# abodthedude25/Ray_Tracing_Octrees

Hardware: AMD Instinct MI355X
Metric: Mrays/s (primary rays), 1920x1080 (higher is better)
Workload: dtype f32

## Files before the change

### ray_tracing_octrees_amd/csrc/rto_device.hip.h

```cpp
#pragma once

#include <hip/hip_runtime.h>
#include <stdint.h>

#include "../../include/rto_hip.h"

namespace rto {

constexpr int kMaxTraversalSteps = 512;
constexpr int kWave = 64;
#ifndef RTO_BLOCK
#define RTO_BLOCK 256
#endif
constexpr int kBlock = RTO_BLOCK;
#ifndef RTO_PACKED3_WAVES
#define RTO_PACKED3_WAVES 6
#endif
#ifndef RTO_PERSIST_CHUNK
#define RTO_PERSIST_CHUNK 8
#endif
constexpr int kMaxDepth = 20;
constexpr int kStackCap = 7 * kMaxDepth + 1;

struct StartState {
// ... 819 lines not shown
    int lvl = 0;
    unsigned lvlPending = 0;
    unsigned tailRun = 0;

#if defined(RTO_STAMP)
    unsigned long long stampSum[5] = { 0, 0, 0, 0, 0 };
#define RTO_T(i) do { __builtin_amdgcn_sched_barrier(0); unsigned long long t_; asm volatile("s_memtime %0\n\ts_waitcnt lgkmcnt(0)" : "=s"(t_) :: "memory"); __builtin_amdgcn_sched_barrier(0); stampSum[i] += t_ - stampLast; stampLast = t_; } while (0)
    unsigned long long stampLast;
    asm volatile("s_memtime %0\n\ts_waitcnt lgkmcnt(0)" : "=s"(stampLast) :: "memory");
#else
#define RTO_T(i) do { } while (0)
#endif
    int trips = 0;
    while (alive) {
        trips++;
        if (MODE == kModeTimeline) tlIters++;
        RTO_T(4);
        const uint2 d = desc[cur];
        const int L = 31 - __builtin_clz(lvlPending | 1u);
        const uint2 e = stk[L * kWave];
        const int half = 1 << (P.depth - 1 - lvl);
        unsigned passMask;
        if (anyRisky) passMask = child_pass_mask<true>(P, r, cx, cy, cz, half);
        else passMask = child_pass_mask_fast(P, r, cx, cy, cz, half);
        RTO_T(0);
        const unsigned vm0 = __builtin_amdgcn_ubfe(d.x, 16, 8);
        const unsigned im0 = __builtin_amdgcn_ubfe(d.x, 8, 8);
        const unsigned sm = d.x & vm0;
        unsigned cand = ((im0 & vm0) | sm) & passMask;
#if defined(RTO_STAMP)
        asm volatile("" :: "v"(cand));
#endif
        RTO_T(1);
        const unsigned solidHit = sm & passMask;
        cand &= 0xffffffffu << (31 - __builtin_clz(solidHit | 1u));
        const bool noWork = cand == 0;
        const int stepsB = steps + __builtin_popcount(vm0) + (int)tailRun;
        const bool dead = noWork && (lvlPending == 0 || stepsB >= kMaxTraversalSteps);
        steps = noWork ? stepsB : steps;
        const unsigned W = noWork ? e.x : ((d.x & 0x00ffff00u) | cand | (tailRun << 24));
        const unsigned base = noWork ? e.y : d.y;
#if defined(RTO_STAMP)
        asm volatile("" :: "v"(W), "v"(base));
#endif
        RTO_T(2);
        const int lvl2 = noWork ? L : lvl;
        const int bpos = P.depth - 1 - lvl2;
        const unsigned childIdx = ((cx >> bpos) & 1) | (((cy >> bpos) & 1) << 1) | (((cz >> bpos) & 1) << 2);
        const unsigned belowPrev = noWork ? ((1u << childIdx) - 1u) : 0xffu;
        const int keep = (int)(0xffffffffu << (bpos + 1));
        cx &= keep; cy &= keep; cz &= keep;
        const unsigned pending = W & 0xffu;
        const unsigned im = __builtin_amdgcn_ubfe(W, 8, 8);
        const unsigned vm = __builtin_amdgcn_ubfe(W, 16, 8);
        const unsigned tailAbove = W >> 24;
        const int j = 31 - __builtin_clz(pending | 1u);
        const unsigned bitj = 1u << j;
        const int stepsC = steps + __builtin_popcount(vm & belowPrev & ~((bitj << 1) - 1u));
        const bool capped = stepsC >= kMaxTraversalSteps;
        const bool go = !dead && !capped;
        const bool solid = (im & bitj) == 0;
        steps = dead ? steps : (capped ? kMaxTraversalSteps : stepsC + 1);
        hit = go && solid;
        const bool descend = go && !solid;
        if (descend) stk[lvl2 * kWave] = make_uint2(W ^ bitj, base);
        const unsigned pendingNew = pending ^ bitj;
        const unsigned lb = 1u << lvl2;
        tailRun = pendingNew ? 0u : tailAbove + (unsigned)__builtin_popcount(vm & (bitj - 1u));
        lvlPending = pendingNew ? (lvlPending | lb) : (lvlPending & ~lb);
        cur = base + (unsigned)__builtin_popcount(im & (bitj - 1u));
        const int hl = 1 << bpos;
        cx |= (j & 1) ? hl : 0; cy |= (j & 2) ? hl : 0; cz |= (j & 4) ? hl : 0;
        lvl = lvl2 + 1;
        alive = descend;
#if defined(RTO_STAMP)
        asm volatile("" :: "v"(cur), "v"(cx), "v"(lvlPending), "v"(tailRun));
#endif
        RTO_T(3);
    }
    if (!hit && steps > kMaxTraversalSteps) steps = kMaxTraversalSteps;
    trips = __builtin_amdgcn_readlane(wave_scan_max_nonneg(trips), kWave - 1);
    if (P.tileCost && lane == 0 && ty < P.tilesY) P.tileCost[tile] = trips;

    const bool mine = valid && !(P.skipOutside && outsideRoot);
    if (MODE == kModeShade) {
        if (mine) __builtin_nontemporal_store(hit ? shade_term(P, r, cx, cy, cz, P.rootSize >> lvl) : kShadeMiss, reinterpret_cast<float*>(out) + (size_t)ly * P.W + px);
        fill_outside<MODE>(P, out, lane, slot);
    } else if (MODE == kModeColor || MODE == kModeTimeline) {
        if (mine) {
            float4 color = make_float4(0.f, 0.f, 0.f, 1.f);
            if (hit) color = shade_hit(P, r, cx, cy, cz, P.rootSize >> lvl);
            store_pixel(out + (size_t)ly * P.W + px, color);
        }
        fill_outside<MODE>(P, out, lane, slot);
        if (MODE == kModeTimeline) {
            int it = tlIters;
            for (int off = 32; off > 0; off >>= 1) it = max(it, __shfl_down(it, off));
            int act = __builtin_popcountll(__builtin_amdgcn_ballot_w64(tlIters > 0));
            if (lane == 0 && ty < P.tilesY) {
                const unsigned long long tl1 = wall_clock64();
                unsigned hwid = __builtin_amdgcn_s_getreg((4 << 0) | (0 << 6) | (31 << 11));
                unsigned xcc = __builtin_amdgcn_s_getreg((20 << 0) | (0 << 6) | (3 << 11));
                int* rec = stepsOut + (size_t)tile * 8;
                rec[0] = (int)(tl0 & 0xffffffffu); rec[1] = (int)(tl0 >> 32);
                rec[2] = (int)(tl1 & 0xffffffffu); rec[3] = (int)(tl1 >> 32);
                rec[4] = it; rec[5] = (int)hwid; rec[6] = (int)xcc; rec[7] = act;
#if defined(RTO_STAMP)
                rec[0] = (int)stampSum[0]; rec[1] = (int)stampSum[1]; rec[5] = (int)stampSum[2]; rec[6] = (int)stampSum[3]; rec[7] = (int)stampSum[4];
#endif
            }
        }
    } else {
        if (inImage) stepsOut[(size_t)py * P.W + px] = hit ? steps : -steps;
        wave_accumulate(counters, steps, hit, inImage);
    }
}

template <int MODE>
__global__ __launch_bounds__(kBlock, RTO_PACKED3_WAVES) void k_trace_packed3(RenderParams P, const uint2* __restrict__ desc,
                                                           float4* __restrict__ out, int* __restrict__ stepsOut,
                                                           Counters* __restrict__ counters) {
    extern __shared__ uint2 lds_stack[];
    const int lane = threadIdx.x & 63;
    const int wave = threadIdx.x >> 6;
    uint2* stk = lds_stack + (size_t)wave * P.depth * kWave + lane;
    const int slot = __builtin_amdgcn_readfirstlane(blockIdx.x * (kBlock / kWave) + wave);
    if (slot >= P.launchWaves) return;
    trace_tile_packed3<MODE>(P, desc, out, stepsOut, counters, stk, lane, slot);
}


template <int TT> __device__ __forceinline__ unsigned bop3(unsigned a, unsigned b, unsigned c) { return __builtin_amdgcn_bitop3_b32(a, b, c, TT); }
constexpr int kSelC = 0xD8;
constexpr int kAndOr = 0xEA;
constexpr int kOrAnd = 0xF8;
constexpr int kAndAndNot = 0x40;
constexpr int kReplace = 0x74;

constexpr unsigned kCoordBias = 0x4B000000u;
template <bool BIASED>
__device__ __forceinline__ void child_axis_terms(float g, float o, float inv, unsigned sgn, int c, float fh, float vs, float sv,
                                                 float& n0, float& n1, float& f0, float& f1) {
    const float fc = BIASED ? __uint_as_float((unsigned)c) - 8388608.0f : (float)c;
    const f32x2 fcc = (f32x2){ fc, fc } + (f32x2){ 0.0f, fh };
    const f32x2 lo = (f32x2){ g, g } + fcc * vs;
    const f32x2 hi = lo + sv;
    const f32x2 t1 = (lo - o) * inv;
    const f32x2 t2 = (hi - o) * inv;
    const unsigned a1x = __float_as_uint(t1.x), a2x = __float_as_uint(t2.x), a1y = __float_as_uint(t1.y), a2y = __float_as_uint(t2.y);
    n0 = __uint_as_float(bop3<kSelC>(a1x, a2x, sgn)); f0 = __uint_as_float(bop3<kSelC>(a2x, a1x, sgn));
    n1 = __uint_as_float(bop3<kSelC>(a1y, a2y, sgn)); f1 = __uint_as_float(bop3<kSelC>(a2y, a1y, sgn));
}

template <bool BIASED>
__device__ __forceinline__ void child_axis_terms_exact(float g, float o, float inv, unsigned sgn, int c, float fh, float vs, float sv,
                                                       float& n0, float& n1, float& f0, float& f1) {
    (void)fh;
    const float fc = BIASED ? __uint_as_float((unsigned)c) - 8388608.0f : (float)c;
    const float p0 = __builtin_fmaf(fc, vs, g);
    const float p1 = p0 + sv;
    const float p2 = p1 + sv;
    const f32x2 t01 = ((f32x2){ p0, p1 } - o) * inv;
    const float t2 = (p2 - o) * inv;
    const unsigned a0 = __float_as_uint(t01.x), a1 = __float_as_uint(t01.y), a2 = __float_as_uint(t2);
    n0 = __uint_as_float(bop3<kSelC>(a0, a1, sgn)); f0 = __uint_as_float(bop3<kSelC>(a1, a0, sgn));
    n1 = __uint_as_float(bop3<kSelC>(a1, a2, sgn)); f1 = __uint_as_float(bop3<kSelC>(a2, a1, sgn));
}

template <bool FOLD = true, bool BIASED = false, bool EXACT = false>
__device__ __forceinline__ unsigned child_fail_mask_fast(float gx, float gy, float gz, float vs, float ox, float oy, float oz,
                                                         float ix, float iy, float iz, unsigned sx, unsigned sy, unsigned sz,
                                                         int cx, int cy, int cz, float fh,
                                                         float clampLo = __uint_as_float(1u), float clampHi = __uint_as_float(0x7149f2c9u)) {
    const float sv = fh * vs;
    const float kEps = clampLo;
    const float kBelow1e30 = clampHi;
    float nx0, nx1, fx0, fx1, ny0, ny1, fy0, fy1, nz0, nz1, fz0, fz1;
    if (EXACT) {
        child_axis_terms_exact<BIASED>(gx, ox, ix, sx, cx, fh, vs, sv, nx0, nx1, fx0, fx1);
        child_axis_terms_exact<BIASED>(gy, oy, iy, sy, cy, fh, vs, sv, ny0, ny1, fy0, fy1);
        child_axis_terms_exact<BIASED>(gz, oz, iz, sz, cz, fh, vs, sv, nz0, nz1, fz0, fz1);
    } else {
        child_axis_terms<BIASED>(gx, ox, ix, sx, cx, fh, vs, sv, nx0, nx1, fx0, fx1);
        child_axis_terms<BIASED>(gy, oy, iy, sy, cy, fh, vs, sv, ny0, ny1, fy0, fy1);
        child_axis_terms<BIASED>(gz, oz, iz, sz, cz, fh, vs, sv, nz0, nz1, fz0, fz1);
    }
    if (FOLD) {
        asm("v_max_f32 %0, %1, %2" : "=v"(nx0) : "v"(nx0), "v"(kEps));
        asm("v_max_f32 %0, %1, %2" : "=v"(nx1) : "v"(nx1), "v"(kEps));
        asm("v_min_f32 %0, %1, %2" : "=v"(fx0) : "v"(fx0), "v"(kBelow1e30));
        asm("v_min_f32 %0, %1, %2" : "=v"(fx1) : "v"(fx1), "v"(kBelow1e30));
    }
#define RTO_D(kx, ky, kz) __float_as_uint(min3f(fx##kx, fy##ky, fz##kz) - max3f(nx##kx, ny##ky, nz##kz))
    unsigned fa = 0, fb = 0;
    fa = __builtin_amdgcn_alignbit(fa, RTO_D(1, 1, 1), 31); fb = __builtin_amdgcn_alignbit(fb, RTO_D(1, 1, 0), 31);
    fa = __builtin_amdgcn_alignbit(fa, RTO_D(0, 1, 1), 31); fb = __builtin_amdgcn_alignbit(fb, RTO_D(0, 1, 0), 31);
    fa = __builtin_amdgcn_alignbit(fa, RTO_D(1, 0, 1), 31); fb = __builtin_amdgcn_alignbit(fb, RTO_D(1, 0, 0), 31);
    fa = __builtin_amdgcn_alignbit(fa, RTO_D(0, 0, 1), 31); fb = __builtin_amdgcn_alignbit(fb, RTO_D(0, 0, 0), 31);
#undef RTO_D
    return (fa << 4) | fb;
}

struct ExactPat { unsigned kaX, kaY, kaZ, xXY, xXZ, xYZ; };
__device__ __forceinline__ ExactPat exact_patterns(unsigned sgnX, unsigned sgnY, unsigned sgnZ) {
    ExactPat p;
    p.kaX = 0xAAu ^ (sgnX & 0xFFu); p.kaY = 0xCCu ^ (sgnY & 0xFFu); p.kaZ = 0xF0u ^ (sgnZ & 0xFFu);
    p.xXY = p.kaX ^ p.kaY; p.xXZ = p.kaX ^ p.kaZ; p.xYZ = p.kaY ^ p.kaZ;
    return p;
}
constexpr int kOr3 = 0xFE;
template <bool BIASED>
__device__ __forceinline__ void axis_emx_exact(float g, float o, float inv, unsigned sgn, int c, float vs, float sv, float& e, float& m, float& x) {
    const float fc = BIASED ? __uint_as_float((unsigned)c) - 8388608.0f : (float)c;
    const float p0 = __builtin_fmaf(fc, vs, g);
    const float p1 = p0 + sv;
    const float p2 = p1 + sv;
    const f32x2 t02 = ((f32x2){ p0, p2 } - o) * inv;
    m = (p1 - o) * inv;
    const unsigned a0 = __float_as_uint(t02.x), a2 = __float_as_uint(t02.y);
    e = __uint_as_float(bop3<kSelC>(a0, a2, sgn)); x = __uint_as_float(bop3<kSelC>(a2, a0, sgn));
}
__device__ __forceinline__ unsigned fails_le(float u, float v) { return (unsigned)((int)__float_as_uint(v - u) >> 31); }

template <bool FOLD, bool BIASED>
__device__ __forceinline__ unsigned child_fail_mask_exactgrid(float gx, float gy, float gz, float vs, float ox, float oy, float oz,
                                                              float ix, float iy, float iz, unsigned sx, unsigned sy, unsigned sz, const ExactPat& K,
                                                              int cx, int cy, int cz, float fh,
                                                              float clampLo = __uint_as_float(1u), float clampHi = __uint_as_float(0x7149f2c9u)) {
    const float sv = fh * vs;
    float ex, mx, xx, ey, my, xy, ez, mz, xz;
    axis_emx_exact<BIASED>(gx, ox, ix, sx, cx, vs, sv, ex, mx, xx);
    axis_emx_exact<BIASED>(gy, oy, iy, sy, cy, vs, sv, ey, my, xy);
    axis_emx_exact<BIASED>(gz, oz, iz, sz, cz, vs, sv, ez, mz, xz);
    float Tn = max3f(ex, ey, ez), Tf = min3f(xx, xy, xz);
    if (FOLD) {
        asm("v_max_f32 %0, %1, %2" : "=v"(Tn) : "v"(Tn), "v"(clampLo));
        asm("v_min_f32 %0, %1, %2" : "=v"(Tf) : "v"(Tf), "v"(clampHi));
    }
    const unsigned selX = bop3<kSelC>(fails_le(Tn, mx), fails_le(mx, Tf), K.kaX);
    const unsigned selY = bop3<kSelC>(fails_le(Tn, my), fails_le(my, Tf), K.kaY);
    const unsigned selZ = bop3<kSelC>(fails_le(Tn, mz), fails_le(mz, Tf), K.kaZ);
    unsigned fail = bop3<kOr3>(selX, selY, selZ);
    const unsigned pXY = bop3<kSelC>(fails_le(my, mx), fails_le(mx, my), K.kaX);
    const unsigned pXZ = bop3<kSelC>(fails_le(mz, mx), fails_le(mx, mz), K.kaX);
    const unsigned pYZ = bop3<kSelC>(fails_le(mz, my), fails_le(my, mz), K.kaY);
    fail = bop3<kOrAnd>(fail, pXY, K.xXY);
    fail = bop3<kOrAnd>(fail, pXZ, K.xXZ);
    fail = bop3<kOrAnd>(fail, pYZ, K.xYZ);
    return fail;
}

struct ExactPat3 { unsigned pack; };
__device__ __forceinline__ ExactPat3 exact_patterns3(unsigned sgnX, unsigned sgnY, unsigned sgnZ) {
    ExactPat3 p;
    p.pack = (0xAAu ^ (sgnX & 0xFFu)) | ((0xCCu ^ (sgnY & 0xFFu)) << 8) | ((0xF0u ^ (sgnZ & 0xFFu)) << 16);
    return p;
}
constexpr int kAndXor = 0x60;
template <bool FOLD, bool BIASED>
__device__ __forceinline__ unsigned child_fail_mask_exactgrid3(float gx, float gy, float gz, float vs, float ox, float oy, float oz,
                                                               float ix, float iy, float iz, const ExactPat3& K,
                                                               int cx, int cy, int cz, float fh,
                                                               float clampLo = __uint_as_float(1u), float clampHi = __uint_as_float(0x7149f2c9u)) {
    const float sv = fh * vs;
    const unsigned sx = (unsigned)((int)__float_as_uint(ix) >> 31), sy = (unsigned)((int)__float_as_uint(iy) >> 31), sz = (unsigned)((int)__float_as_uint(iz) >> 31);
    float ex, mx, xx, ey, my, xy, ez, mz, xz;
    axis_emx_exact<BIASED>(gx, ox, ix, sx, cx, vs, sv, ex, mx, xx);
    axis_emx_exact<BIASED>(gy, oy, iy, sy, cy, vs, sv, ey, my, xy);
    axis_emx_exact<BIASED>(gz, oz, iz, sz, cz, vs, sv, ez, mz, xz);
    float Tn = max3f(ex, ey, ez), Tf = min3f(xx, xy, xz);
    if (FOLD) {
        asm("v_max_f32 %0, %1, %2" : "=v"(Tn) : "v"(Tn), "v"(clampLo));
        asm("v_min_f32 %0, %1, %2" : "=v"(Tf) : "v"(Tf), "v"(clampHi));
    }
    const unsigned kaX = K.pack, kaY = K.pack >> 8, kaZ = K.pack >> 16;
    const unsigned selX = bop3<kSelC>(fails_le(Tn, mx), fails_le(mx, Tf), kaX);
    const unsigned selY = bop3<kSelC>(fails_le(Tn, my), fails_le(my, Tf), kaY);
    const unsigned selZ = bop3<kSelC>(fails_le(Tn, mz), fails_le(mz, Tf), kaZ);
    const unsigned pXY = bop3<kAndXor>(bop3<kSelC>(fails_le(my, mx), fails_le(mx, my), kaX), kaX, kaY);
    const unsigned pXZ = bop3<kAndXor>(bop3<kSelC>(fails_le(mz, mx), fails_le(mx, mz), kaX), kaX, kaZ);
    const unsigned pYZ = bop3<kAndXor>(bop3<kSelC>(fails_le(mz, my), fails_le(my, mz), kaY), kaY, kaZ);
    return bop3<kOr3>(selX, selY, selZ) | bop3<kOr3>(pXY, pXZ, pYZ);
}

__device__ __forceinline__ unsigned child_fail_mask_exact(float gx, float gy, float gz, float vs, float ox, float oy, float oz,
                                                       float ix, float iy, float iz, int cx, int cy, int cz, int half) {
    const float sv = (float)half * vs;
    unsigned fail = 0;
#pragma unroll 1
    for (int k = 0; k < 8; k++) {
        const float mnx = gx + (float)(cx + ((k & 1) ? half : 0)) * vs;
        const float mny = gy + (float)(cy + ((k & 2) ? half : 0)) * vs;
        const float mnz = gz + (float)(cz + ((k & 4) ? half : 0)) * vs;
        const float t1x = (mnx - ox) * ix, t1y = (mny - oy) * iy, t1z = (mnz - oz) * iz;
        const float t2x = ((mnx + sv) - ox) * ix, t2y = ((mny + sv) - oy) * iy, t2z = ((mnz + sv) - oz) * iz;
        const float tn = gmax(gmax(gmin(t1x, t2x), gmin(t1y, t2y)), gmin(t1z, t2z));
        const float tf = gmin(gmin(gmax(t1x, t2x), gmax(t1y, t2y)), gmax(t1z, t2z));
        const bool ok = (tn <= tf) && (tf > 0.0f) && !(tn >= 1e30f);
        fail |= ok ? 0u : (1u << k);
    }
    return fail;
}

template <int MODE, int EXACT = -1>
__device__ __forceinline__ void trace_tile_lean(const RenderParams& P, const uint2* __restrict__ desc, float4* __restrict__ out,
                                                int* __restrict__ stepsOut, Counters* __restrict__ counters, uint2* stk,
                                                const int lane, const int slot) {
    unsigned long long tl0 = 0;
    if (MODE == kModeTimeline) tl0 = wall_clock64();

    int tile, tx, ty;
    resolve_slot(P, slot, tx, ty, tile);
    const int px = tx * 8 + (lane & 7);
    const int ly = ty * 8 + (lane >> 3);
    const bool valid = (ty < P.tilesY) && (px < P.W) && (ly < P.localRows);
    const int py = global_row(P, ly);
    const bool inImage = valid && (py < P.H);

    const Geo G = geo_of(P);
    bool hit = false;
    int steps0 = 0;
    Ray r;
    bool alive = false;
    const bool outsideRoot = px < P.rootX0 || px > P.rootX1 || py < P.rootY0 || py > P.rootY1;
    bool guarded = false;
    int startVisible = P.rootVisible, startShift = P.depth, startSize = P.rootSize, startX = 0, startY = 0, startZ = 0;
    unsigned startDesc = 0;
    bool startLeaf = false, startSolid = false;
    if (P.start) {
        const StartState st = *P.start;
        startVisible = st.visible; startShift = st.shift; startSize = 1 << st.shift; startX = st.x; startY = st.y; startZ = st.z;
        startDesc = st.desc; startLeaf = st.leaf != 0; startSolid = st.solid != 0;
    }
    const bool tileLive = tile_may_hit(P, tx, ty, slot, lane, tile);
    if (inImage && startVisible && tileLive) {
        steps0 = 1;
        if (!outsideRoot) {
            r = generate_ray_tab(P, px, py);
            float tNear, tFar, a0, a1, a2, a3, a4, a5;
            alive = slab_exact(G, r, startX, startY, startZ, startSize, tNear, tFar, a0, a1, a2, a3, a4, a5) && !(tNear >= 1e30f);
            const float reach = 0x1p-20f * gmax(gmax(gmax(__builtin_fabsf(a0), __builtin_fabsf(a3)), __builtin_fabsf(r.ox)) * __builtin_fabsf(r.ix),
                                                gmax(gmax(gmax(__builtin_fabsf(a1), __builtin_fabsf(a4)), __builtin_fabsf(r.oy)) * __builtin_fabsf(r.iy),
                                                     gmax(gmax(__builtin_fabsf(a2), __builtin_fabsf(a5)), __builtin_fabsf(r.oz)) * __builtin_fabsf(r.iz)));
            guarded = alive && !(tNear > reach && tNear * 1024.0f >= tFar && tFar < 1e29f);
        }
    }
    const bool risky = alive && !(__builtin_isfinite(r.ix) && __builtin_isfinite(r.iy) && __builtin_isfinite(r.iz) &&
                                  __builtin_isfinite(r.ox) && __builtin_isfinite(r.oy) && __builtin_isfinite(r.oz));
    const bool anyRisky = __builtin_amdgcn_ballot_w64(risky) != 0ull;
    const bool plainWave = __builtin_amdgcn_ballot_w64(guarded) == 0ull;
    const bool exactGrid = EXACT < 0 ? P.exactGrid != 0 : EXACT != 0;
    float gxv = G.gx, gyv = G.gy, gzv = G.gz;
    asm volatile("" : "+v"(gxv), "+v"(gyv), "+v"(gzv));

    unsigned cur = startDesc;
    int cx = (int)(kCoordBias | (unsigned)startX), cy = (int)(kCoordBias | (unsigned)startY), cz = (int)(kCoordBias | (unsigned)startZ);
    int bpos = startShift - 1;
    unsigned lvlPending = 0;
    const unsigned sentinel = 1u << P.depth;
    int S = 0;
    const int capBound = kMaxTraversalSteps + 7 * P.depth;
    const unsigned sgnX = (unsigned)((int)__float_as_uint(r.ix) >> 31), sgnY = (unsigned)((int)__float_as_uint(r.iy) >> 31),
                   sgnZ = (unsigned)((int)__float_as_uint(r.iz) >> 31);
    const ExactPat K = exact_patterns(sgnX, sgnY, sgnZ);
    const char* descBytes = reinterpret_cast<const char*>(desc);
    int trips = 0;
    if (startLeaf) { hit = alive && startSolid; alive = false; }
    while (alive) {
        trips++;
        const uint2 d = *reinterpret_cast<const uint2*>(descBytes + (cur << 3));
        const int Lb = __builtin_ctz(lvlPending | sentinel);
        const uint2 e = stk[Lb * kWave];
        const float fh = __uint_as_float((unsigned)(bpos + 127) << 23);
        unsigned fail8;
        if (anyRisky) fail8 = child_fail_mask_exact(G.gx, G.gy, G.gz, G.vs, r.ox, r.oy, r.oz,
                                                    r.ix, r.iy, r.iz, cx & 0x7fffff, cy & 0x7fffff, cz & 0x7fffff, 1 << bpos);
        else if (exactGrid) {
            if (plainWave) fail8 = child_fail_mask_exactgrid<false, true>(gxv, gyv, gzv, G.vs, r.ox, r.oy, r.oz, r.ix, r.iy, r.iz,
                                                                          sgnX, sgnY, sgnZ, K, cx, cy, cz, fh);
            else fail8 = child_fail_mask_exactgrid<true, true>(gxv, gyv, gzv, G.vs, r.ox, r.oy, r.oz, r.ix, r.iy, r.iz,
                                                               sgnX, sgnY, sgnZ, K, cx, cy, cz, fh);
        }
        else if (plainWave) fail8 = child_fail_mask_fast<false, true>(G.gx, G.gy, G.gz, G.vs, r.ox, r.oy, r.oz, r.ix, r.iy, r.iz,
                                                                      sgnX, sgnY, sgnZ, cx, cy, cz, fh);
        else fail8 = child_fail_mask_fast<true, true>(G.gx, G.gy, G.gz, G.vs, r.ox, r.oy, r.oz, r.ix, r.iy, r.iz,
                                                      sgnX, sgnY, sgnZ, cx, cy, cz, fh);
        const unsigned vm0 = (d.x >> 16) & 0xffu;
        S += __builtin_popcount(vm0);
        const unsigned cand = bop3<kAndAndNot>(d.x | (d.x >> 8), vm0, fail8);
        const unsigned noWork = (unsigned)(((int)cand - 1) >> 31);
        const bool dead = (cand | lvlPending) == 0 || S >= capBound;
        const unsigned W = bop3<kSelC>(bop3<kAndOr>(d.x, 0x00ffff00u, cand), e.x, noWork);
        const unsigned base = bop3<kSelC>(d.y, e.y, noWork);
        const int bpos2 = (int)bop3<kSelC>((unsigned)bpos, (unsigned)Lb, noWork);
        const int j = 31 - __builtin_clz(W & 0xffu);
        const unsigned bitj = 0x80000000u >> (31 - j);
        const unsigned imv = W >> 8;
        const bool solid = (imv & bitj) == 0;
        hit = !dead && solid;
        const unsigned Wn = W ^ bitj;
        stk[bpos2 * kWave] = make_uint2(Wn, base);
        const unsigned hl = 1u << bpos2;
        const unsigned noneLeft = (unsigned)(((int)(Wn & 0xffu) - 1) >> 31);
        lvlPending = bop3<kReplace>(lvlPending, hl, noneLeft);
        cur = base + (unsigned)__builtin_popcount(imv & (bitj - 1u));
        const unsigned keep = 0u - (hl + hl);
        const unsigned sj = (unsigned)j << bpos2;
        cx = (int)bop3<kOrAnd>((unsigned)cx & keep, sj, hl);
        cy = (int)bop3<kOrAnd>((unsigned)cy & keep, sj >> 1, hl);
        cz = (int)bop3<kOrAnd>((unsigned)cz & keep, sj >> 2, hl);
        bpos = bpos2 - 1;
        alive = !dead && !solid;
    }
    if (P.tileCost || MODE == kModeTimeline) {
        trips = __builtin_amdgcn_readlane(wave_scan_max_nonneg(trips), kWave - 1);
        if (P.tileCost && lane == 0 && ty < P.tilesY && tileLive) P.tileCost[tile] = (trips == 0 && P.tileMask) ? -1 : trips;
    }
    const int leafShift = bpos + 1;
    cx &= 0x7fffff; cy &= 0x7fffff; cz &= 0x7fffff;

    int steps = steps0 + S;
    if (hit && (MODE == kModeSteps || steps > kMaxTraversalSteps)) {
        int R = 0;
        for (int b = startShift - 1; b > bpos; b--) {
            const unsigned w = stk[b * kWave].x;
            const unsigned jl = ((cx >> b) & 1) | (((cy >> b) & 1) << 1) | (((cz >> b) & 1) << 2);
            R += __builtin_popcount(__builtin_amdgcn_ubfe(w, 16, 8) & ((1u << jl) - 1u));
        }
        steps -= R;
        if (steps > kMaxTraversalSteps) hit = false;
    }
    if (steps > kMaxTraversalSteps) steps = kMaxTraversalSteps;

    const bool mine = valid && !(P.skipOutside && outsideRoot);
    if (MODE == kModeShade) {
        if (mine) __builtin_nontemporal_store(hit ? shade_term(P, G, r, cx, cy, cz, 1 << leafShift) : kShadeMiss, reinterpret_cast<float*>(out) + (size_t)ly * P.W + px);
        fill_outside<MODE>(P, out, lane, slot);
    } else if (MODE == kModeColor || MODE == kModeTimeline) {
        if (mine) {
            float4 color = make_float4(0.f, 0.f, 0.f, 1.f);
            if (hit) color = shade_color(shade_term(P, G, r, cx, cy, cz, 1 << leafShift));
            store_pixel(out + (size_t)ly * P.W + px, color);
        }
        fill_outside<MODE>(P, out, lane, slot);
        if (MODE == kModeTimeline) {
            const int act = __builtin_popcountll(__builtin_amdgcn_ballot_w64(steps0 + S > 1));
            if (lane == 0 && ty < P.tilesY) {
                const unsigned long long tl1 = wall_clock64();
                unsigned hwid = __builtin_amdgcn_s_getreg((4 << 0) | (0 << 6) | (31 << 11));
                unsigned xcc = __builtin_amdgcn_s_getreg((20 << 0) | (0 << 6) | (3 << 11));
                int* rec = stepsOut + (size_t)tile * 8;
                rec[0] = (int)(tl0 & 0xffffffffu); rec[1] = (int)(tl0 >> 32);
                rec[2] = (int)(tl1 & 0xffffffffu); rec[3] = (int)(tl1 >> 32);
                rec[4] = trips; rec[5] = (int)hwid; rec[6] = (int)xcc; rec[7] = act | (slot << 8);
            }
        }
    } else {
        if (inImage) stepsOut[(size_t)py * P.W + px] = hit ? steps : -steps;
        wave_accumulate(counters, steps, hit, inImage);
    }
}

template <int MODE>
__global__ __launch_bounds__(kBlock) void k_closest_lean(RenderParams P, const uint2* __restrict__ desc, float4* __restrict__ out,
                                                          Counters* __restrict__ counters) {
    extern __shared__ uint2 lds_stack[];
    const int lane = threadIdx.x & 63, wave = threadIdx.x >> 6;
    uint2* stk = lds_stack + (size_t)wave * (P.depth + 1) * kWave + lane;
    const int tile = blockIdx.x * (kBlock / kWave) + wave;
    const int tx = tile % P.tilesX, ty = tile / P.tilesX;
    const int px = tx * 8 + (lane & 7), ly = ty * 8 + (lane >> 3);
    const bool valid = (ty < P.tilesY) && (px < P.W) && (ly < P.localRows);
    const int py = global_row(P, ly);
    const bool inImage = valid && (py < P.H);
    const Geo G = geo_of(P);

    bool hit = false, active = false, enter = false;
    long long entered = 0;
    int steps0 = 0;
    float closestT = 1e30f;
    int bx = 0, by = 0, bz = 0, bs = 0;
    Ray r;
    r.ox = r.oy = r.oz = r.dx = r.dy = r.dz = r.ix = r.iy = r.iz = 0.0f;
    if (inImage && P.rootVisible) {
        steps0 = 1;
        r = generate_ray_tab(P, px, py);
        float tNear, tFar, a0, a1, a2, a3, a4, a5;
        active = enter = slab_exact(G, r, 0, 0, 0, P.rootSize, tNear, tFar, a0, a1, a2, a3, a4, a5) && !(tNear >= closestT);
    }
    unsigned cur = 0, lvlPending = 0;
    int cx = 0, cy = 0, cz = 0, bpos = P.depth - 1;
    while (active) {
        if (enter) {
            entered++;
            const uint2 d = desc[cur];
            const unsigned fail8 = child_fail_mask_exact(G.gx, G.gy, G.gz, G.vs, r.ox, r.oy, r.oz, r.ix, r.iy, r.iz, cx, cy, cz, 1 << bpos);
            const unsigned im = (d.x >> 8) & 0xffu;
            const unsigned cand = ((d.x | im) & 0xffu) & ~fail8;
            stk[bpos * kWave] = make_uint2(cand | (im << 8), d.y);
            lvlPending = cand ? (lvlPending | (1u << bpos)) : (lvlPending & ~(1u << bpos));
            enter = false;
        }
        if (lvlPending == 0) break;
        const int Lb = __builtin_ctz(lvlPending);
        const uint2 e = stk[Lb * kWave];
        const int j = 31 - __builtin_clz(e.x & 0xffu);
        const unsigned bit = 1u << j, left = e.x ^ bit;
        stk[Lb * kWave].x = left;
        if ((left & 0xffu) == 0) lvlPending &= ~(1u << Lb);
        const int h = 1 << Lb, keep = ~(2 * h - 1);
        const int chx = (cx & keep) + ((j & 1) ? h : 0), chy = (cy & keep) + ((j & 2) ? h : 0), chz = (cz & keep) + ((j & 4) ? h : 0);
        float tNear, tFar, a0, a1, a2, a3, a4, a5;
        const bool pass = slab_exact(G, r, chx, chy, chz, h, tNear, tFar, a0, a1, a2, a3, a4, a5);
        if (pass && !(tNear >= closestT)) {
            const unsigned im = (e.x >> 8) & 0xffu;
            if (im & bit) {
                cur = e.y + (unsigned)__builtin_popcount(im & (bit - 1u));
                cx = chx; cy = chy; cz = chz; bpos = Lb - 1; enter = true;
            } else {
                const float tHit = gmax(0.0f, tNear);
                if (tHit < closestT && tHit <= tFar) { closestT = tHit; hit = true; bx = chx; by = chy; bz = chz; bs = h; }
            }
        }
    }
    const float shade = hit ? shade_term(P, G, r, bx, by, bz, bs) : kShadeMiss;
    if (valid) out[(size_t)ly * P.W + px] = shade_color(shade);
    if (MODE == kModeSteps) {
        unsigned long long pops = inImage ? (unsigned long long)(steps0 + 8 * entered) : 0ull, hits = (inImage && hit) ? 1ull : 0ull;
        for (int off = 32; off > 0; off >>= 1) { pops += __shfl_down(pops, off); hits += __shfl_down(hits, off); }
        if (lane == 0) { atomicAdd(&counters->pops, pops); atomicAdd(&counters->hits, hits); }
    }
}

__device__ __forceinline__ bool pops_before(int ax, int ay, int az, int bx, int by, int bz) {
    const unsigned m = (unsigned)((ax ^ bx) | (ay ^ by) | (az ^ bz));
    if (m == 0) return false;
    const int top = 31 - __builtin_clz(m);
    const int ja = ((ax >> top) & 1) | (((ay >> top) & 1) << 1) | (((az >> top) & 1) << 2);
    const int jb = ((bx >> top) & 1) | (((by >> top) & 1) << 1) | (((bz >> top) & 1) << 2);
#ifdef RTO_TEST_WRONG_TIE
    return ja < jb;
#else
    return ja > jb;
#endif
}
__device__ __forceinline__ unsigned flip_children(unsigned m, unsigned flip) {
    if (flip & 1u) m = ((m & 0x55u) << 1) | ((m >> 1) & 0x55u);
    if (flip & 2u) m = ((m & 0x33u) << 2) | ((m >> 2) & 0x33u);
    if (flip & 4u) m = ((m & 0x0fu) << 4) | ((m >> 4) & 0x0fu);
    return m;
}
__global__ __launch_bounds__(kBlock) void k_closest_near_first(RenderParams P, const uint2* __restrict__ desc, float4* __restrict__ out) {
    extern __shared__ uint2 lds_stack[];
    const int lane = threadIdx.x & 63, wave = threadIdx.x >> 6;
    if ((int)blockIdx.x < P.maskBlocks) { mask_block(P, (int)blockIdx.x, reinterpret_cast<unsigned*>(lds_stack), P.maskLdsBytes >> 2); return; }
    const int slot = __builtin_amdgcn_readfirstlane(((int)blockIdx.x - P.maskBlocks) * (kBlock / kWave) + wave);
    if (slot >= P.launchWaves) return;
    uint2* stk = lds_stack + (size_t)wave * (P.depth + 1) * kWave + lane;
    int tile, tx, ty;
    resolve_slot(P, slot, tx, ty, tile);
    const int px = tx * 8 + (lane & 7), ly = ty * 8 + (lane >> 3);
    const bool valid = (ty < P.tilesY) && (px < P.W) && (ly < P.localRows);
    const int py = global_row(P, ly);
    const bool inImage = valid && (py < P.H);
    const bool outside = px < P.rootX0 || px > P.rootX1 || py < P.rootY0 || py > P.rootY1;
    const bool tileLive = tile_may_hit(P, tx, ty, slot, lane, tile);
    const Geo G = geo_of(P);

    bool hit = false, active = false, enter = false;
    float best = 1e30f;
    int bx = 0, by = 0, bz = 0, bs = 0;
    unsigned flip = 0;
    Ray r;
    r.ox = r.oy = r.oz = r.dx = r.dy = r.dz = r.ix = r.iy = r.iz = 0.0f;
    if (inImage && P.rootVisible && !outside && tileLive) {
        r = generate_ray_tab(P, px, py);
        flip = (r.dx < 0.0f ? 1u : 0u) | (r.dy < 0.0f ? 2u : 0u) | (r.dz < 0.0f ? 4u : 0u);
        float tNear, tFar, a0, a1, a2, a3, a4, a5;
        active = enter = slab_exact(G, r, 0, 0, 0, P.rootSize, tNear, tFar, a0, a1, a2, a3, a4, a5) && !(tNear >= 1e30f);
    }
    const bool risky = active && !(__builtin_isfinite(r.ix) && __builtin_isfinite(r.iy) && __builtin_isfinite(r.iz) &&
                                   __builtin_isfinite(r.ox) && __builtin_isfinite(r.oy) && __builtin_isfinite(r.oz));
    const bool anyRisky = __builtin_amdgcn_ballot_w64(risky) != 0ull;
    const unsigned sgnX = (unsigned)((int)__float_as_uint(r.ix) >> 31), sgnY = (unsigned)((int)__float_as_uint(r.iy) >> 31),
                   sgnZ = (unsigned)((int)__float_as_uint(r.iz) >> 31);
    const float kBelow1e30 = __uint_as_float(0x7149f2c9u);
    unsigned cur = 0, lvlPending = 0;
    int cx = 0, cy = 0, cz = 0, bpos = P.depth - 1;
    int entered = 0;
    while (active) {
        if (enter) {
            entered++;
            const uint2 d = desc[cur];
            unsigned fail8;
            if (anyRisky) fail8 = child_fail_mask_exact(G.gx, G.gy, G.gz, G.vs, r.ox, r.oy, r.oz, r.ix, r.iy, r.iz, cx, cy, cz, 1 << bpos);
            else fail8 = child_fail_mask_fast<true, false>(G.gx, G.gy, G.gz, G.vs, r.ox, r.oy, r.oz, r.ix, r.iy, r.iz, sgnX, sgnY, sgnZ, cx, cy, cz,
                                                           (float)(1 << bpos), __uint_as_float(1u), gmax(__uint_as_float(1u), gmin(best, kBelow1e30)));
            const unsigned im = (d.x >> 8) & 0xffu;
            const unsigned cand = flip_children(((d.x | im) & 0xffu) & ~fail8, flip);
            stk[bpos * kWave] = make_uint2(cand | (im << 8), d.y);
            lvlPending = cand ? (lvlPending | (1u << bpos)) : (lvlPending & ~(1u << bpos));
            enter = false;
        }
        if (lvlPending == 0) break;
        const int Lb = __builtin_ctz(lvlPending);
        const uint2 e = stk[Lb * kWave];
        const int i = __builtin_ctz(e.x & 0xffu);
        const unsigned left = e.x ^ (1u << i);
        stk[Lb * kWave].x = left;
        if ((left & 0xffu) == 0) lvlPending &= ~(1u << Lb);
        const int j = i ^ (int)flip;
        const unsigned bit = 1u << j;
        const int h = 1 << Lb, keep = ~(2 * h - 1);
        const int chx = (cx & keep) + ((j & 1) ? h : 0), chy = (cy & keep) + ((j & 2) ? h : 0), chz = (cz & keep) + ((j & 4) ? h : 0);
        float tNear, tFar, a0, a1, a2, a3, a4, a5;
        const bool pass = slab_exact(G, r, chx, chy, chz, h, tNear, tFar, a0, a1, a2, a3, a4, a5);
        if (pass && !(tNear >= 1e30f) && !(tNear > best)) {
            const unsigned im = (e.x >> 8) & 0xffu;
            if (im & bit) {
                cur = e.y + (unsigned)__builtin_popcount(im & (bit - 1u));
                cx = chx; cy = chy; cz = chz; bpos = Lb - 1; enter = true;
            } else {
                const float tHit = gmax(0.0f, tNear);
                const bool nearer = tHit < best;
                const bool tie = tHit == best;
                const bool first = pops_before(chx, chy, chz, bx, by, bz);
                if (tHit <= tFar && (nearer || (tie && first))) {
                    best = tHit; hit = true; bx = chx; by = chy; bz = chz; bs = h;
                }
            }
        }
    }
    if (P.tileCost && tileLive) {
        const int cost = __builtin_amdgcn_readlane(wave_scan_max_nonneg(entered), kWave - 1);
        if (lane == 0 && ty < P.tilesY) P.tileCost[tile] = (cost == 0 && P.tileMask) ? -1 : (cost + 3) >> 2;
    }
    const float shade = hit ? shade_term(P, G, r, bx, by, bz, bs) : kShadeMiss;
    if (valid && !(P.skipOutside && outside)) store_pixel(out + (size_t)ly * P.W + px, shade_color(shade));
    fill_outside<kModeColor>(P, out, lane, slot);
}

#ifndef RTO_LEAN_WAVES
#define RTO_LEAN_WAVES 6
#endif
template <int MODE, int EXACT>
__global__ __launch_bounds__(kBlock, RTO_LEAN_WAVES) void k_trace_lean(RenderParams P, const uint2* __restrict__ desc,
                                                           float4* __restrict__ out, int* __restrict__ stepsOut,
                                                           Counters* __restrict__ counters) {
    extern __shared__ uint2 lds_stack[];
    const int lane = threadIdx.x & 63;
    const int wave = threadIdx.x >> 6;
    uint2* stk = lds_stack + (size_t)wave * (P.depth + 1) * kWave + lane;
    if ((int)blockIdx.x < P.maskBlocks) { mask_block(P, (int)blockIdx.x, reinterpret_cast<unsigned*>(lds_stack), P.maskLdsBytes >> 2); return; }
    const int slot = __builtin_amdgcn_readfirstlane(((int)blockIdx.x - P.maskBlocks) * (int)(blockDim.x >> 6) + wave);
    if (slot >= P.launchWaves) return;
    trace_tile_lean<MODE, EXACT>(P, desc, out, stepsOut, counters, stk, lane, slot);
}

constexpr int kMaxBatch = 8;
struct RenderBatch {
    RenderParams P[kMaxBatch];
    float4* out[kMaxBatch];
    int n;
};
template <int MODE, int EXACT>
__global__ __launch_bounds__(kBlock, RTO_LEAN_WAVES) void k_trace_lean_batch(RenderBatch B, const uint2* __restrict__ desc) {
    extern __shared__ uint2 lds_stack[];
    const int lane = threadIdx.x & 63;
    const int wave = threadIdx.x >> 6;
    const int mb = B.P[0].maskBlocks;
    if ((int)blockIdx.x < mb * B.n) { const int fm = (int)blockIdx.x / mb; mask_block(B.P[fm], (int)blockIdx.x - fm * mb, reinterpret_cast<unsigned*>(lds_stack), B.P[fm].maskLdsBytes >> 2); return; }
    const int g = __builtin_amdgcn_readfirstlane(((int)blockIdx.x - mb * B.n) * (int)(blockDim.x >> 6) + wave);
    const int slot = g / B.n, f = g - slot * B.n;
    const RenderParams& P = B.P[f];
    uint2* stk = lds_stack + (size_t)wave * (P.depth + 1) * kWave + lane;
    if (slot >= P.launchWaves) return;
    trace_tile_lean<MODE, EXACT>(P, desc, B.out[f], nullptr, nullptr, stk, lane, slot);
}

#ifndef RTO_PERSIST_WAVES
#define RTO_PERSIST_WAVES 5
#endif
template <int MODE>
__global__ __launch_bounds__(kBlock, RTO_PERSIST_WAVES) void k_trace_lean_persistent(RenderParams P, const uint2* __restrict__ desc,
                                                           float4* __restrict__ out, int* __restrict__ stepsOut,
                                                           Counters* __restrict__ counters, int* __restrict__ queue) {
    extern __shared__ uint2 lds_stack[];
    const int lane = threadIdx.x & 63;
    const int wave = threadIdx.x >> 6;
    uint2* stk = lds_stack + (size_t)wave * (P.depth + 1) * kWave + lane;
    const int tiles = P.launchWaves;
    const int firstFree = gridDim.x * (kBlock / kWave);
    int slot = __builtin_amdgcn_readfirstlane(blockIdx.x * (kBlock / kWave) + wave);
    int left = 1;
    while (slot < tiles) {
        trace_tile_lean<MODE>(P, desc, out, stepsOut, counters, stk, lane, slot);
        slot++;
        if (--left == 0) {
            int next = 0;
            if (lane == 0) next = atomicAdd(queue, kPersistChunk);
            slot = firstFree + __builtin_amdgcn_readfirstlane(next);
            left = kPersistChunk;
        }
    }
}

struct CullParams {
    float planes[24];
    float gridMin[3];
    float voxelSize;
    float margin;
};

__device__ __forceinline__ bool node_visible(const CullParams& C, int x, int y, int z, int size) {
    float mn[3] = { C.gridMin[0] + (float)x * C.voxelSize, C.gridMin[1] + (float)y * C.voxelSize,
// ... 2141 lines not shown
```

Before: 77470.

## Split traversal loop into main phase and specialized tail for few live lanes

The lean traversal loop now exits its general path once the number of still-active lanes in the wave drops to a small threshold, using a scalar popcount of the ballot. The remaining lanes finish in a simplified tail loop that always uses the plain exact-grid child test and adds an early termination bound based on an upper estimate of steps. This is meant to cut per-iteration overhead during the divergent tail where only a few lanes work. It adds a second loop copy, which raises code size and register pressure, and it changes how the step-cap cutoff is applied.

After: 73500. 0.949x the previous value.

```diff
diff --git a/ray_tracing_octrees_amd/csrc/rto_device.hip.h b/ray_tracing_octrees_amd/csrc/rto_device.hip.h
--- a/ray_tracing_octrees_amd/csrc/rto_device.hip.h
+++ b/ray_tracing_octrees_amd/csrc/rto_device.hip.h
@@ -1145,6 +1145,20 @@
     return fail;
 }
 
+#ifndef RTO_TAIL_LANES
+#define RTO_TAIL_LANES 4
+#endif
+constexpr int kTailLanes = RTO_TAIL_LANES;
+template <bool TAIL>
+__device__ __forceinline__ bool lean_loop_goes_on(bool alive, int handOver) {
+    if (!TAIL) return alive;
+    const unsigned long long live = __builtin_amdgcn_ballot_w64(alive);
+    unsigned long long go;
+    int count;
+    asm("s_bcnt1_i32_b64 %1, %2\n\ts_cmp_gt_i32 %1, %3\n\ts_cselect_b64 %0, %2, 0" : "=s"(go), "=&s"(count) : "s"(live), "s"(handOver) : "scc");
+    return __builtin_amdgcn_inverse_ballot_w64(go);
+}
+
 template <int MODE, int EXACT = -1>
 __device__ __forceinline__ void trace_tile_lean(const RenderParams& P, const uint2* __restrict__ desc, float4* __restrict__ out,
                                                 int* __restrict__ stepsOut, Counters* __restrict__ counters, uint2* stk,
@@ -1209,7 +1223,9 @@
     const char* descBytes = reinterpret_cast<const char*>(desc);
     int trips = 0;
     if (startLeaf) { hit = alive && startSolid; alive = false; }
-    while (alive) {
+    constexpr bool kTail = EXACT != 0 && kTailLanes > 0;
+    const int handOver = (kTail && exactGrid && plainWave && !anyRisky) ? kTailLanes : 0;
+    if (lean_loop_goes_on<kTail>(alive, handOver)) do {
         trips++;
         const uint2 d = *reinterpret_cast<const uint2*>(descBytes + (cur << 3));
         const int Lb = __builtin_ctz(lvlPending | sentinel);
@@ -1254,6 +1270,46 @@
         cz = (int)bop3<kOrAnd>((unsigned)cz & keep, sj >> 2, hl);
         bpos = bpos2 - 1;
         alive = !dead && !solid;
+    } while (lean_loop_goes_on<kTail>(alive, handOver));
+    if (kTail) {
+        const unsigned pathMask = (1u << startShift) - 1u;
+        while (alive) {
+            trips++;
+            const uint2 d = *reinterpret_cast<const uint2*>(descBytes + (cur << 3));
+            const int Lb = __builtin_ctz(lvlPending | sentinel);
+            const uint2 e = stk[Lb * kWave];
+            const float fh = __uint_as_float((unsigned)(bpos + 127) << 23);
+            const unsigned fail8 = child_fail_mask_exactgrid<false, true>(gxv, gyv, gzv, G.vs, r.ox, r.oy, r.oz, r.ix, r.iy, r.iz,
+                                                                          sgnX, sgnY, sgnZ, K, cx, cy, cz, fh);
+            const unsigned vm0 = (d.x >> 16) & 0xffu;
+            S += __builtin_popcount(vm0);
+            const unsigned cand = bop3<kAndAndNot>(d.x | (d.x >> 8), vm0, fail8);
+            const unsigned noWork = (unsigned)(((int)cand - 1) >> 31);
+            const bool dead = (cand | lvlPending) == 0;
+            const unsigned W = bop3<kSelC>(bop3<kAndOr>(d.x, 0x00ffff00u, cand), e.x, noWork);
+            const unsigned base = bop3<kSelC>(d.y, e.y, noWork);
+            const int bpos2 = (int)bop3<kSelC>((unsigned)bpos, (unsigned)Lb, noWork);
+            const int j = 31 - __builtin_clz(W & 0xffu);
+            const unsigned bitj = 0x80000000u >> (31 - j);
+            const unsigned imv = W >> 8;
+            const bool solid = (imv & bitj) == 0;
+            hit = !dead && solid;
+            const unsigned Wn = W ^ bitj;
+            stk[bpos2 * kWave] = make_uint2(Wn, base);
+            const unsigned hl = 1u << bpos2;
+            const unsigned noneLeft = (unsigned)(((int)(Wn & 0xffu) - 1) >> 31);
+            lvlPending = bop3<kReplace>(lvlPending, hl, noneLeft);
+            cur = base + (unsigned)__builtin_popcount(imv & (bitj - 1u));
+            const unsigned keep = 0u - (hl + hl);
+            const unsigned sj = (unsigned)j << bpos2;
+            cx = (int)bop3<kOrAnd>((unsigned)cx & keep, sj, hl);
+            cy = (int)bop3<kOrAnd>((unsigned)cy & keep, sj >> 1, hl);
+            cz = (int)bop3<kOrAnd>((unsigned)cz & keep, sj >> 2, hl);
+            bpos = bpos2 - 1;
+            const unsigned pm = pathMask & (0u - hl);
+            const int Rub = __builtin_popcount((unsigned)cx & pm) + 2 * (__builtin_popcount((unsigned)cy & pm) + 2 * __builtin_popcount((unsigned)cz & pm));
+            alive = !dead && !solid && S - Rub < kMaxTraversalSteps;
+        }
     }
     if (P.tileCost || MODE == kModeTimeline) {
         trips = __builtin_amdgcn_readlane(wave_scan_max_nonneg(trips), kWave - 1);
```
